# guptakhil/show-tell

Hardware: AMD Instinct MI355X
Metric: training images/sec (ResNet101+GRU, emb=512, bs=128) at 1/2/4/8 MI355X (higher is better)
Workload: dtype bf16; 1 GPU; BASELINE configs[1]: ResNet-101 (train-mode BN, frozen) + 5-layer GRU decoder, E=H=512, V=10000, fwd+bwd+SGD step, synthetic COCO-shaped batch; batch_per_gpu=128, global_batch=128, image=3x224x224, parallelism=dp1

## Files before the change

include/showtell_hip.h:

```cpp
#ifndef SHOWTELL_HIP_H
#define SHOWTELL_HIP_H

#include <stddef.h>
#include <stdint.h>

#ifdef __cplusplus
extern "C" {
#endif

#define ST_F32 0
#define ST_BF16 1

#define ST_CELL_GRU 0
#define ST_CELL_LSTM 1

const char* st_last_error(void);
int st_version(void);

typedef struct {
  const void* x;
  const void* w;
  void* y;
  const float* bias;
  const float* scale;
  const float* shift;
  const void* residual;
  float* stats;
  int dtype, out_dtype;
  int B, Hin, Win, Cin, Ho, Wo, N, KH, KW, stride, pad;
  int ldx, ldw, ldy;
  int relu, accumulate;
  int Cin_logical;
  int k_order;
  int stats_replicas;
  const float* in_stats; const float* in_gamma; const float* in_beta; float in_count, in_eps;
  int split_k;
} st_conv_desc;

int st_conv(const st_conv_desc* d, void* stream);
int st_conv_batch(const st_conv_desc* d, int n, void* stream);

typedef struct {
  const void* a;
  const void* b;
  float* c;
  const int* b_row;
  const int* b_live;
  float* colsum0;
  float* colsum1;
  int dtype;
  int M, N, K;
  int lda, ldb, ldc;
  int accumulate;
} st_gemm_tn_desc;
int st_gemm_tn_batch(const st_gemm_tn_desc* d, int n, void* stream);

typedef struct {
  const void* x; const void* w_frag; void* y;
  float* stats; int stats_replicas;
  const float* scale; const float* shift; int relu;
  const float* in_stats; const float* in_gamma; const float* in_beta; float in_count; float in_eps;
  int B, H, W, C, N;
  int in_stats_replicas;
} st_conv3x3_img_desc;
int st_conv3x3_img_supported(int H, int W, int C, int N);
int st_conv3x3_img(const st_conv3x3_img_desc* d, void* stream);
int st_conv3x3_s2_supported(int C, int N);
int st_conv3x3_s2(const st_conv3x3_img_desc* d, void* stream);
typedef struct {
  const void* x; const void* w_frag; void* y; const void* residual;
  float* stats; int stats_replicas;
  const float* scale; const float* shift; int relu;
  const float* in_stats; const float* in_gamma; const float* in_beta; float in_count; float in_eps; int in_stats_replicas;
  int B, Hin, Win, C, N, stride;
} st_conv1x1_wreg_desc;
int st_conv1x1_wreg_supported(int C, int N);
int st_conv1x1_wreg(const st_conv1x1_wreg_desc* d, void* stream);
int st_conv1x1_kstream_supported(int C, int N);
int st_conv1x1_kstream(const st_conv1x1_wreg_desc* d, void* stream);
typedef struct {
  const void* raw; const void* identity; void* x_out; const void* w_frag; void* y;
  float* stats; int stats_replicas;
  const float* f_stats; const float* f_gamma; const float* f_beta; float f_count; float f_eps; int f_stats_replicas;
  long rows; int C, N;
  const float* id_stats; const float* id_gamma; const float* id_beta; int id_stats_replicas;
} st_conv1x1_kfuse_desc;
int st_conv1x1_kfuse_supported(int C, int N);
int st_conv1x1_kfuse(const st_conv1x1_kfuse_desc* d, void* stream);
#ifdef ST_EXPERIMENTAL
int st_conv1x1_kfuse8(const st_conv1x1_kfuse_desc* d, void* stream);
#endif
typedef struct {
  const void* raw2; const void* w3_frag; const void* identity; void* x_out; const void* w1_frag; void* y;
  float* stats; int stats_replicas;
  const float* bn2_stats; const float* bn2_gamma; const float* bn2_beta; int bn2_replicas;
  const float* bn3_stats; const float* bn3_gamma; const float* bn3_beta; int bn3_replicas;
  const float* id_stats; const float* id_gamma; const float* id_beta; int id_replicas;
  float count; float eps;
  long rows; int C1, C2, N;
} st_conv_b2b_desc;
int st_conv_b2b_supported(int C1, int C2, int N);
int st_conv_b2b(const st_conv_b2b_desc* d, void* stream);
typedef struct {
  const void* x2; const void* w3_frag; const void* identity; void* x_out; const void* w1_frag; void* y;
  float* stats; int stats_replicas;
  const float* bn2_stats; const float* bn2_gamma; const float* bn2_beta; int bn2_replicas;
  const float* bn3_stats; const float* bn3_gamma; const float* bn3_beta; int bn3_replicas;
  float count; float eps;
  const float* scale3; const float* shift3; const float* scale1; const float* shift1; int relu1;
  long rows; int C1, C2, N;
  const float* id_stats; const float* id_gamma; const float* id_beta; int id_replicas;
} st_conv_c3c1_desc;
int st_conv_c3c1_supported(int C1, int C2, int N);
int st_conv_c3c1(const st_conv_c3c1_desc* d, void* stream);
int st_conv1x1_astat_supported(int C, int N);
int st_conv1x1_astat(const st_conv1x1_wreg_desc* d, void* stream);

int st_pack_conv_weight_frag(const float* w, void* out, int Cout, int Cin, int KH, int KW, int ntw, void* stream);

int st_tune(int reserved, int kc, int w8);
int st_prof_enable(int on);
int st_debug_stamps(unsigned long long* buf);
int st_prof_collect(double* ms, double* flops, long* launches);

typedef struct {
  const void* x; void* y; const void* res;
  const float* stats;  const float* gamma; const float* beta;
  const float* running_mean; const float* running_var;
  const float* res_stats; const float* res_gamma; const float* res_beta;
  const float* res_running_mean; const float* res_running_var;
  int res_bn;
  int dtype; long rows; int C; float count; float eps; int relu;
  int stats_replicas, res_stats_replicas;
} st_bn_act_desc;

int st_bn_act(const st_bn_act_desc* d, void* stream);

int st_bn_update_running(const float* stats, float* running_mean, float* running_var,
// ... 255 lines not shown
```

show-tell_amd/_lib.py:

```python
import ctypes as C
import os

import torch

_HERE = os.path.dirname(os.path.abspath(__file__))
LIB_PATH = os.path.join(_HERE, "lib", "libshowtell_hip.so")

ST_F32, ST_BF16 = 0, 1
ST_CELL_GRU, ST_CELL_LSTM = 0, 1

c_p, c_i, c_f, c_l = C.c_void_p, C.c_int, C.c_float, C.c_long


class ConvDesc(C.Structure):
    _fields_ = [("x", c_p), ("w", c_p), ("y", c_p), ("bias", c_p), ("scale", c_p), ("shift", c_p),
                ("residual", c_p), ("stats", c_p), ("dtype", c_i), ("out_dtype", c_i),
                ("B", c_i), ("Hin", c_i), ("Win", c_i), ("Cin", c_i), ("Ho", c_i), ("Wo", c_i), ("N", c_i),
                ("KH", c_i), ("KW", c_i), ("stride", c_i), ("pad", c_i),
                ("ldx", c_i), ("ldw", c_i), ("ldy", c_i), ("relu", c_i), ("accumulate", c_i), ("Cin_logical", c_i), ("k_order", c_i), ("stats_replicas", c_i),
                ("in_stats", c_p), ("in_gamma", c_p), ("in_beta", c_p), ("in_count", c_f), ("in_eps", c_f), ("split_k", c_i)]


class Conv3x3ImgDesc(C.Structure):
    _fields_ = [("x", c_p), ("w_frag", c_p), ("y", c_p), ("stats", c_p), ("stats_replicas", c_i), ("scale", c_p), ("shift", c_p),
# ... 19 lines not shown
                ("scale", c_p), ("shift", c_p), ("B", c_i), ("H", c_i), ("W", c_i)]


class ConvB2bDesc(C.Structure):
    _fields_ = [("raw2", c_p), ("w3_frag", c_p), ("identity", c_p), ("x_out", c_p), ("w1_frag", c_p), ("y", c_p),
                ("stats", c_p), ("stats_replicas", c_i),
                ("bn2_stats", c_p), ("bn2_gamma", c_p), ("bn2_beta", c_p), ("bn2_replicas", c_i),
                ("bn3_stats", c_p), ("bn3_gamma", c_p), ("bn3_beta", c_p), ("bn3_replicas", c_i),
                ("id_stats", c_p), ("id_gamma", c_p), ("id_beta", c_p), ("id_replicas", c_i),
                ("count", c_f), ("eps", c_f), ("rows", c_l), ("C1", c_i), ("C2", c_i), ("N", c_i)]


class ConvC3c1Desc(C.Structure):
    _fields_ = [("x2", c_p), ("w3_frag", c_p), ("identity", c_p), ("x_out", c_p), ("w1_frag", c_p), ("y", c_p),
                ("stats", c_p), ("stats_replicas", c_i),
                ("bn2_stats", c_p), ("bn2_gamma", c_p), ("bn2_beta", c_p), ("bn2_replicas", c_i),
                ("bn3_stats", c_p), ("bn3_gamma", c_p), ("bn3_beta", c_p), ("bn3_replicas", c_i),
                ("count", c_f), ("eps", c_f),
                ("scale3", c_p), ("shift3", c_p), ("scale1", c_p), ("shift1", c_p), ("relu1", c_i),
                ("rows", c_l), ("C1", c_i), ("C2", c_i), ("N", c_i),
                ("id_stats", c_p), ("id_gamma", c_p), ("id_beta", c_p), ("id_replicas", c_i)]


class BnActDesc(C.Structure):
    _fields_ = [("x", c_p), ("y", c_p), ("res", c_p), ("stats", c_p), ("gamma", c_p), ("beta", c_p),
                ("running_mean", c_p), ("running_var", c_p), ("res_stats", c_p), ("res_gamma", c_p),
                ("res_beta", c_p), ("res_running_mean", c_p), ("res_running_var", c_p), ("res_bn", c_i),
                ("dtype", c_i), ("rows", c_l), ("C", c_i), ("count", c_f), ("eps", c_f), ("relu", c_i),
                ("stats_replicas", c_i), ("res_stats_replicas", c_i)]


ST_MAX_LAYERS = 8


class RnnParams(C.Structure):
    _fields_ = [("cell", c_i), ("dtype", c_i), ("L", c_i), ("in0", c_i), ("H", c_i), ("V", c_i), ("E", c_i),
                ("emb", c_p), ("w_ih", c_p * ST_MAX_LAYERS), ("w_hh", c_p * ST_MAX_LAYERS),
                ("b_ih", c_p * ST_MAX_LAYERS), ("b_hh", c_p * ST_MAX_LAYERS), ("w_lin", c_p), ("b_lin", c_p)]


class RnnGrads(C.Structure):
    _fields_ = [("emb", c_p), ("w_ih", c_p * ST_MAX_LAYERS), ("w_hh", c_p * ST_MAX_LAYERS),
                ("b_ih", c_p * ST_MAX_LAYERS), ("b_hh", c_p * ST_MAX_LAYERS), ("w_lin", c_p), ("b_lin", c_p)]


class AttnParams(C.Structure):
    _fields_ = [("rnn", RnnParams), ("F", c_i), ("A", c_i), ("P", c_i),
                ("w_enc", c_p), ("b_enc", c_p), ("w_dec", c_p), ("b_dec", c_p), ("w_full", c_p), ("b_full", c_p),
                ("w_init_h", c_p), ("b_init_h", c_p), ("w_init_c", c_p), ("b_init_c", c_p), ("w_embed", c_p), ("b_embed", c_p)]


class AttnGrads(C.Structure):
    _fields_ = [("rnn", RnnGrads)] + [(n, c_p) for n in ("w_enc", "b_enc", "w_dec", "b_dec", "w_full", "b_full", "w_init_h", "b_init_h",
                                                        "w_init_c", "b_init_c", "w_embed", "b_embed")]


class PackedSeq(C.Structure):
    _fields_ = [("B", c_i), ("T", c_i), ("ntok", c_i), ("Tcap", c_i), ("batch_sizes_host", C.POINTER(c_i)),
                ("rows_b", c_p), ("rows_t", c_p), ("prev_row", c_p), ("caption", c_p)]


class DropoutDesc(C.Structure):
    _fields_ = [("p_in", C.c_double), ("p_layer", C.c_double), ("p_out", C.c_double), ("seed", c_l), ("step", c_i),
                ("buf", c_p), ("buf_bytes", C.c_size_t)]


class LossTerms(C.Structure):
    _fields_ = [("row_weight", c_p), ("nll_out", c_p), ("smoothing", c_i), ("label_smoothing", c_f), ("smooth_out", c_p),
                ("tile_sums", c_p), ("tile_sums_bytes", C.c_size_t)]


class ImageBatchDesc(C.Structure):
    _fields_ = [("src", c_p), ("src_bytes", C.c_int64), ("offset", c_p), ("height", c_p), ("width", c_p), ("flip", c_p), ("batch", c_i),
                ("max_height", c_i), ("max_width", c_i), ("out_h", c_i), ("out_w", c_i), ("lut", c_p), ("tmp", c_p),
                ("out", c_p), ("out_u8", c_p)]


_SIGS = {
    "st_version": ([], c_i),
    "st_image_transform": ([C.POINTER(ImageBatchDesc), c_p], c_i),
    "st_conv": ([C.POINTER(ConvDesc), c_p], c_i),
    "st_conv_batch": ([C.POINTER(ConvDesc), c_i, c_p], c_i),
    "st_gemm_tn_batch": ([c_p, c_i, c_p], c_i),
    "st_conv3x3_img_supported": ([c_i, c_i, c_i, c_i], c_i),
    "st_conv3x3_img": ([C.POINTER(Conv3x3ImgDesc), c_p], c_i),
    "st_conv3x3_s2_supported": ([c_i, c_i], c_i),
    "st_conv3x3_s2": ([C.POINTER(Conv3x3ImgDesc), c_p], c_i),
    "st_conv1x1_wreg_supported": ([c_i, c_i], c_i),
    "st_conv1x1_wreg": ([C.POINTER(Conv1x1WregDesc), c_p], c_i),
    "st_conv1x1_kfuse": ([C.POINTER(Conv1x1KfuseDesc), c_p], c_i),
    "st_conv1x1_kfuse_supported": ([c_i, c_i], c_i),
    "st_conv1x1_kfuse8": ([C.POINTER(Conv1x1KfuseDesc), c_p], c_i),
    "st_conv_b2b": ([C.POINTER(ConvB2bDesc), c_p], c_i),
    "st_conv_b2b_supported": ([c_i, c_i, c_i], c_i),
    "st_conv_c3c1": ([C.POINTER(ConvC3c1Desc), c_p], c_i),
    "st_conv_c3c1_supported": ([c_i, c_i, c_i], c_i),
    "st_conv1x1_astat_supported": ([c_i, c_i], c_i),
    "st_conv1x1_astat": ([C.POINTER(Conv1x1WregDesc), c_p], c_i),
    "st_conv1x1_kstream_supported": ([c_i, c_i], c_i),
    "st_conv1x1_kstream": ([C.POINTER(Conv1x1WregDesc), c_p], c_i),
    "st_pack_conv_weight_frag": ([c_p, c_p, c_i, c_i, c_i, c_i, c_i, c_p], c_i),
    "st_tune": ([c_i, c_i, c_i], c_i),
    "st_prof_enable": ([c_i], c_i),
    "st_debug_stamps": ([c_p], c_i),
    "st_prof_collect": ([C.POINTER(C.c_double), C.POINTER(C.c_double), C.POINTER(c_l)], c_i),
    "st_bn_act": ([C.POINTER(BnActDesc), c_p], c_i),
    "st_bn_update_running": ([c_p, c_p, c_p, c_i, c_f, c_f, c_p], c_i),
    "st_nchw_to_nhwc": ([c_p, c_p, c_i, c_i, c_i, c_i, c_i, c_i, c_p], c_i),
    "st_nchw_to_s2d16": ([c_p, c_p, c_i, c_i, c_i, c_i, c_p], c_i),
    "st_stem_weight_s2d": ([c_p, c_p, c_i, c_i, c_p], c_i),
    "st_stem_weight_frag": ([c_p, c_p, c_p], c_i),
    "st_stem_weight_frag_packed": ([c_p, c_i, c_p, c_p], c_i),
    "st_stem_conv_pool": ([C.POINTER(StemConvPoolDesc), c_p], c_i),
    "st_nhwc_to_ncp_f32": ([c_p, c_p, c_i, c_i, c_i, c_i, c_p], c_i),
    "st_maxpool3x3s2": ([c_p, c_p, c_i, c_i, c_i, c_i, c_i, c_p], c_i),
    "st_maxpool3x3s2_bn": ([c_p, c_p, c_i, c_i, c_i, c_i, c_i, c_p, c_p, c_p, c_p, c_p, c_f, c_f, c_p], c_i),
    "st_global_avgpool": ([c_p, c_p, c_i, c_i, c_i, c_i, c_i, c_p], c_i),
    "st_cast": ([c_p, c_p, c_i, c_i, c_l, c_p], c_i),
    "st_transpose": ([c_p, c_p, c_i, c_i, c_i, c_i, c_i, c_p], c_i),
    "st_transpose_colsum": ([c_p, c_p, c_p, c_i, c_i, c_i, c_i, c_i, c_p], c_i),
    "st_transpose_batch": ([c_p, c_p, c_p, c_i, c_i, c_i, c_i, c_i, c_i, c_p, c_p, c_p], c_i),
    "st_pack_conv_weight": ([c_p, c_p, c_i, c_i, c_i, c_i, c_i, c_i, c_i, c_p], c_i),
    "st_cast2d": ([c_p, c_p, c_i, c_i, c_i, c_i, c_i, c_i, c_p], c_i),
    "st_rnn_vocab_ld": ([c_i], c_i),
    "st_rnn_workspace_bytes": ([C.POINTER(RnnParams), C.POINTER(PackedSeq)], C.c_size_t),
    "st_rnn_forward": ([C.POINTER(RnnParams), C.POINTER(PackedSeq), c_p, c_p, C.c_size_t, c_p, c_i, c_i, c_p, c_i, C.POINTER(DropoutDesc),
                        c_p, c_p], c_i),
    "st_rnn_backward": ([C.POINTER(RnnParams), C.POINTER(RnnGrads), C.POINTER(PackedSeq), c_p, c_i, c_p, C.c_size_t, c_p,
                         C.POINTER(DropoutDesc), c_p, c_p], c_i),
    "st_rnn_fused_loss_supported": ([C.POINTER(RnnParams)], c_i),
    "st_rnn_fused_loss_bytes": ([C.POINTER(RnnParams), C.POINTER(PackedSeq)], C.c_size_t),
    "st_rnn_fused_loss_ls_bytes": ([C.POINTER(RnnParams), C.POINTER(PackedSeq)], C.c_size_t),
    "st_rnn_fused_loss": ([C.POINTER(RnnParams), C.POINTER(PackedSeq), c_p, C.c_size_t, c_p, c_p, C.c_size_t, C.POINTER(LossTerms), c_p,
                           C.POINTER(DropoutDesc), c_p], c_i),
    "st_rnn_fused_dlogits": ([C.POINTER(RnnParams), C.POINTER(PackedSeq), c_p, C.c_size_t, c_p, c_p, c_p, C.POINTER(LossTerms), c_p, c_i,
                              C.POINTER(DropoutDesc), c_p], c_i),
    "st_dropout_rows": ([c_p, c_p, c_i, c_i, c_i, c_i, c_i, C.c_double, c_l, c_i, c_i, c_i, c_p], c_i),
    "st_rnn_dropout_bytes": ([C.POINTER(RnnParams), C.POINTER(PackedSeq)], C.c_size_t),
    "st_rnn_greedy_workspace_bytes": ([C.POINTER(RnnParams), c_i], C.c_size_t),
    "st_rnn_greedy": ([C.POINTER(RnnParams), c_p, c_i, c_i, c_p, C.c_size_t, c_p, c_p, c_p], c_i),
    "st_rnn_greedy_last_route": ([], c_i),
    "st_rnn_step": ([C.POINTER(RnnParams), c_p, c_i, c_p, c_p, c_p, c_p, c_p, c_i, c_p], c_i),
    "st_embedding_rows": ([c_p, c_p, c_p, c_i, c_i, c_i, c_i, c_i, c_p], c_i),
    "st_gather_state": ([c_p, c_p, c_p, c_i, c_i, c_i, c_i, c_i, c_p], c_i),
    "st_softmax_topk": ([c_p, c_i, c_i, c_i, c_i, c_p, c_p, c_i, c_p], c_i),
    "st_beam_select": ([c_p, c_p, c_p, c_p, c_p, c_i, c_i, c_i, c_l, c_p, c_p, c_p, c_p, c_p, c_p], c_i),
    "st_beam_ban_topk": ([c_p, c_i, c_i, c_i, c_i, c_p, c_i, c_i, c_i, c_p, c_i, c_l, c_i, c_p, c_p, c_p], c_i),
    "st_beam_select_hist": ([c_p, c_p, c_p, c_p, c_p, c_i, c_i, c_i, c_l, c_p, c_p, c_p, c_p, c_p, c_p, c_p, c_i, c_i, c_p], c_i),
    "st_sample_rows": ([c_p, c_i, c_i, c_i, c_p, c_i, c_f, c_i, c_l, c_p, c_p, c_p, c_i, c_i, c_p, c_p], c_i),
    "st_rnn_sample_workspace_bytes": ([C.POINTER(RnnParams), c_i], C.c_size_t),
    "st_rnn_sample": ([C.POINTER(RnnParams), c_p, c_i, c_i, c_p, c_f, c_i, c_l, c_p, C.c_size_t, c_p, c_p, c_p], c_i),
    "st_sample_mix_rows": ([c_p, c_i, c_i, c_i, c_p, c_i, c_f, c_i, c_p, c_i, c_f, c_p, c_i, c_l, c_p, c_i, c_p, c_p, c_p, c_p, c_i, c_i, c_p,
                            c_p], c_i),
    "st_rnn_sched_inputs_workspace_bytes": ([C.POINTER(RnnParams), c_i], C.c_size_t),
    "st_rnn_sched_inputs": ([C.POINTER(RnnParams), c_p, c_i, c_p, c_i, c_p, c_i, c_p, c_p, c_f, c_f, c_i, c_p, C.c_size_t, c_p, c_p, c_p, c_p,
                             c_p], c_i),
    "st_attn_workspace_bytes": ([c_p, c_p], C.c_size_t),
    "st_attn_forward": ([c_p, c_p, c_p, c_p, c_p, C.c_size_t, c_p, c_i, c_i, c_p, c_i, C.POINTER(DropoutDesc), c_p], c_i),
    "st_attn_backward": ([c_p, c_p, c_p, c_p, c_p, c_i, c_p, c_p, c_f, c_p, c_p, C.c_size_t, C.POINTER(DropoutDesc), c_p], c_i),
    "st_attn_dropout_bytes": ([c_p, c_p], C.c_size_t),
    "st_attn_reg_loss": ([c_p, c_i, c_i, c_i, c_f, c_p, c_p], c_i),
    "st_attn_greedy_workspace_bytes": ([c_p, c_i], C.c_size_t),
    "st_attn_greedy": ([c_p, c_p, c_i, c_i, c_l, c_p, C.c_size_t, c_p, c_p], c_i),
    "st_attn_greedy_alphas": ([c_p, c_p, c_i, c_i, c_l, c_p, C.c_size_t, c_p, c_p, c_p], c_i),
    "st_attn_sample_workspace_bytes": ([c_p, c_i], C.c_size_t),
    "st_attn_sample": ([c_p, c_p, c_i, c_i, c_l, c_p, c_f, c_i, c_l, c_p, C.c_size_t, c_p, c_p, c_p, c_p], c_i),
# ... 103 lines not shown
```

show-tell_amd/csrc/gemm_tn.hip:

```cpp
#include "common.h"
#include "tn_tile.h"
#include <string.h>
#include <type_traits>

namespace {

constexpr int kMaxGroups = 12;
constexpr int kImages = 2;
constexpr int kStep = kImages * TN_BK;
constexpr int kRowsPerThread = kStep / 16;

struct TnGroup {
  const bf16_t* a; const bf16_t* b; float* c;
  const int* b_row; const int* b_live;
  float* cs0; float* cs1;
  int M, N, K, lda, ldb, ldc, accumulate;
  int tile0, ntn;
};
struct TnArgs { TnGroup g[kMaxGroups]; int ng, ntiles; };

typedef __attribute__((ext_vector_type(4))) short s16x4;
typedef __attribute__((ext_vector_type(8))) short s16x8;
typedef __attribute__((address_space(3))) s16x4 lds_s16x4;

// ... 77 lines not shown
      const int row = r0 + 16 * i;
      const int off = (row / TN_BK) * TN_IMAGE_BYTES + tn_store_off(row % TN_BK, ch);
      *reinterpret_cast<u32x4*>(buf + off) = ra[i];
      *reinterpret_cast<u32x4*>(buf + kImages * TN_IMAGE_BYTES + off) = rb[i];
    }
    if (do_cs) {
#pragma unroll
      for (int i = 0; i < kRowsPerThread; ++i)
#pragma unroll
        for (int e = 0; e < 4; ++e) {
          cs[2 * e] += __uint_as_float(ra[i][e] << 16);
          cs[2 * e + 1] += __uint_as_float(ra[i][e] & 0xffff0000u);
        }
    }
    __syncthreads();
    if (s + 1 < nsteps) {
      load((s + 1) * kStep);
      resolve((s + 2) * kStep);
    }
#pragma unroll
    for (int im = 0; im < kImages; ++im) {
      const char* ia = buf + im * TN_IMAGE_BYTES;
      const char* ib = buf + (kImages + im) * TN_IMAGE_BYTES;
      bf16x8 fa[4], fb[4];
#pragma unroll
      for (int i = 0; i < 4; ++i) { fa[i] = tr_frag(ia, lane, 4 * wm + i); fb[i] = tr_frag(ib, lane, 4 * wn + i); }
#pragma unroll
      for (int i = 0; i < 4; ++i)
#pragma unroll
        for (int j = 0; j < 4; ++j) acc[i][j] = __builtin_amdgcn_mfma_f32_16x16x32_bf16(fa[i], fb[j], acc[i][j], 0, 0, 0);
    }
  }

  float* const cbase = g.c;
  const long ldc = g.ldc;
  const bool accumulate = g.accumulate != 0;
  auto write_c = [&](auto full_tag) {
    constexpr bool kFull = decltype(full_tag)::value;
    float* const cl = cbase + (long)(m0 + 64 * wm + 4 * (lane >> 4)) * ldc + (n0 + 64 * wn + (lane & 15));
#pragma unroll
    for (int i0 = 0; i0 < 4; i0 += 2) {
      float prior[2][4][4];
#pragma unroll
      for (int i = 0; i < 2; ++i)
#pragma unroll
        for (int r = 0; r < 4; ++r)
#pragma unroll
          for (int j = 0; j < 4; ++j) {
            const int m = m0 + 64 * wm + 16 * (i0 + i) + 4 * (lane >> 4) + r, n = n0 + 64 * wn + 16 * j + (lane & 15);
            const bool ok = kFull || (m < M && n < N);
            prior[i][r][j] = 0.f;
            if (accumulate) prior[i][r][j] = ok ? cl[(16 * (i0 + i) + r) * ldc + 16 * j] : 0.f;
          }
#pragma unroll
      for (int i = 0; i < 2; ++i)
#pragma unroll
        for (int r = 0; r < 4; ++r)
#pragma unroll
          for (int j = 0; j < 4; ++j) {
            const int m = m0 + 64 * wm + 16 * (i0 + i) + 4 * (lane >> 4) + r, n = n0 + 64 * wn + 16 * j + (lane & 15);
            if (kFull || (m < M && n < N)) cl[(16 * (i0 + i) + r) * ldc + 16 * j] = prior[i][r][j] + acc[i0 + i][j][r];
          }
    }
  };
  if (m0 + TN_COLS <= M && n0 + TN_COLS <= N) write_c(std::true_type{});
  else write_c(std::false_type{});

  if (do_cs) {
    __syncthreads();
    float* red = reinterpret_cast<float*>(&lds[0][0][0][0]);
#pragma unroll
    for (int e = 0; e < 8; ++e) red[r0 * TN_COLS + 8 * ch + e] = cs[e];
    __syncthreads();
    if (tid < TN_COLS && m0 + tid < M) {
      float sum = 0.f;
#pragma unroll
      for (int r = 0; r < 16; ++r) sum += red[r * TN_COLS + tid];
      if (g.cs0) g.cs0[m0 + tid] += sum;
      if (g.cs1) g.cs1[m0 + tid] += sum;
    }
  }
}

}

extern "C" int st_gemm_tn_batch(const st_gemm_tn_desc* d, int n, void* stream) {
  ST_CHECK(d && n >= 1 && n <= kMaxGroups, "st_gemm_tn_batch: 1..%d problems per launch", kMaxGroups);
  TnArgs args;
  memset(&args, 0, sizeof(args));
  long tiles = 0;
  for (int i = 0; i < n; ++i) {
    const st_gemm_tn_desc& p = d[i];
    ST_CHECK(p.dtype == ST_BF16, "st_gemm_tn_batch: problem %d: bf16 only (the transposed LDS read is a 16-bit one)", i);
    ST_CHECK(p.a && p.b && p.c, "st_gemm_tn_batch: problem %d: null pointer", i);
    ST_CHECK(p.M >= 1 && p.N >= 1 && p.K >= 1, "st_gemm_tn_batch: problem %d: bad shape M=%d N=%d K=%d", i, p.M, p.N, p.K);
    ST_CHECK(p.lda >= p.M && p.ldb >= p.N && p.ldc >= p.N, "st_gemm_tn_batch: problem %d: leading dimension below the extent (lda=%d M=%d ldb=%d N=%d ldc=%d)",
             i, p.lda, p.M, p.ldb, p.N, p.ldc);
    ST_CHECK(p.lda % 8 == 0 && p.ldb % 8 == 0, "st_gemm_tn_batch: problem %d: lda=%d and ldb=%d must be multiples of 8", i, p.lda, p.ldb);
    ST_CHECK(((reinterpret_cast<uintptr_t>(p.a) | reinterpret_cast<uintptr_t>(p.b)) & 15) == 0, "st_gemm_tn_batch: problem %d: a and b must be 16-byte aligned", i);
    ST_CHECK(!p.b_live || p.b_row, "st_gemm_tn_batch: problem %d: b_live goes with b_row", i);
    TnGroup& g = args.g[i];
    g.a = reinterpret_cast<const bf16_t*>(p.a); g.b = reinterpret_cast<const bf16_t*>(p.b); g.c = p.c;
    g.b_row = p.b_row; g.b_live = p.b_live; g.cs0 = p.colsum0; g.cs1 = p.colsum1;
    g.M = p.M; g.N = p.N; g.K = p.K; g.lda = p.lda; g.ldb = p.ldb; g.ldc = p.ldc; g.accumulate = p.accumulate;
    g.tile0 = (int)tiles;
    g.ntn = (p.N + TN_COLS - 1) / TN_COLS;
    tiles += (long)((p.M + TN_COLS - 1) / TN_COLS) * g.ntn;
    ST_CHECK(tiles < (1L << 24), "st_gemm_tn_batch: too many output tiles");
  }
  args.ng = n; args.ntiles = (int)tiles;
  const int grid = (int)((tiles + 7) / 8 * 8);
  hipLaunchKernelGGL(gemm_tn_kernel, dim3(grid), dim3(256), 0, reinterpret_cast<hipStream_t>(stream), args);
  ST_LAUNCH_CHECK();
  return 0;
}
```

show-tell_amd/csrc/rnn.cpp:

```cpp
#include "decoder_host.h"
#include <stdlib.h>

namespace {

struct Plan {
  int G, GH, Np, Vp, maxw;
  size_t es;
  size_t x0, y, gates, cst, dyl, dx0, dgx, dgh, dhc, dcc, tA, tB, wT, wThh, wTih, gA, gB, total;
};

Plan make_plan(const st_rnn_params* p, const st_packed_seq* s) {
  Plan q;
  q.G = p->cell == ST_CELL_GRU ? 3 : 4;
  q.GH = q.G * p->H;
  q.Np = st_up8(s->ntok);
  q.Vp = st_rnn_vocab_ld(p->V);
  q.es = st_dtype_size(p->dtype);
  q.maxw = p->in0 > p->H ? p->in0 : p->H;
  const size_t n = s->ntok, L = p->L, H = p->H;
  Arena ar;
  q.x0 = ar.take(n * p->in0 * q.es);
  q.y = ar.take(L * n * H * q.es);
  q.gates = ar.take(L * n * 4 * H * q.es);
  q.cst = ar.take(p->cell == ST_CELL_LSTM ? L * n * H * q.es : 0);
// ... 115 lines not shown
namespace {
int fused_rows(const st_rnn_params* p, const st_packed_seq* s, const void* workspace, size_t workspace_bytes, const st_loss_terms* t,
               const st_dropout* drop, const char* who, const char** ytop) {
  if (check_common(p, s, who)) return 1;
  if (st_check_loss_terms(t, who)) return 1;
  ST_CHECK(st_rnn_fused_loss_supported(p), "%s: needs bf16, H = 512 and the vocabulary projection (use st_rnn_forward's logits + st_cross_entropy)", who);
  const Plan q = make_plan(p, s);
  ST_CHECK(workspace, "%s: null pointer", who);
  ST_CHECK(workspace_bytes >= q.total, "%s: workspace / scratch too small", who);
  DropPlan dp;
  if (st_drop_plan(drop, p->L, s->ntok, p->H, p->dtype, false, who, &dp)) return 1;
  *ytop = dp.out ? dp.rows(p->L - 1) : reinterpret_cast<const char*>(workspace) + q.y + (size_t)(p->L - 1) * s->ntok * p->H * q.es;
  return 0;
}
}

extern "C" int st_rnn_fused_loss(const st_rnn_params* p, const st_packed_seq* s, const void* workspace, size_t workspace_bytes,
                                 const long* targets, float* scratch, size_t scratch_bytes, const st_loss_terms* terms, float* loss_accum,
                                 const st_dropout* drop, void* stream) {
  const st_loss_terms t = terms ? *terms : st_loss_terms{};
  const char* ytop;
  if (fused_rows(p, s, workspace, workspace_bytes, &t, drop, "st_rnn_fused_loss", &ytop)) return 1;
  ST_CHECK(targets && scratch && (loss_accum || t.nll_out || t.smooth_out) && (t.tile_sums || !t.smoothing), "st_rnn_fused_loss: null pointer");
  ST_CHECK(scratch_bytes >= st_rnn_fused_loss_bytes(p, s), "st_rnn_fused_loss: workspace / scratch too small");
  ST_CHECK(!t.smoothing || t.tile_sums_bytes >= st_rnn_fused_loss_ls_bytes(p, s), "st_rnn_fused_loss: tile_sums too small (%zu < %zu)",
           t.tile_sums_bytes, st_rnn_fused_loss_ls_bytes(p, s));
  const int n = s->ntok;
  return vocab_ce_forward(ytop, p->w_lin, p->b_lin, targets, n, p->V, scratch + 2 * (size_t)n, scratch + n, scratch, loss_accum, t.row_weight,
                          t.nll_out, reinterpret_cast<hipStream_t>(stream), t.tile_sums, t.smooth_out, t.label_smoothing);
}
extern "C" int st_rnn_fused_dlogits(const st_rnn_params* p, const st_packed_seq* s, const void* workspace, size_t workspace_bytes,
                                    const long* targets, const float* scratch, const float* grad_scale_dev, const st_loss_terms* terms,
                                    void* dlogits, int ldd, const st_dropout* drop, void* stream) {
  const st_loss_terms t = terms ? *terms : st_loss_terms{};
  const char* ytop;
  if (fused_rows(p, s, workspace, workspace_bytes, &t, drop, "st_rnn_fused_dlogits", &ytop)) return 1;
  ST_CHECK(targets && scratch && dlogits, "st_rnn_fused_dlogits: null pointer");
  return vocab_ce_dlogits(ytop, p->w_lin, p->b_lin, targets, scratch, s->ntok, p->V, dlogits, ldd, 1.0f, grad_scale_dev, t.row_weight,
                          reinterpret_cast<hipStream_t>(stream), t.smoothing != 0, t.label_smoothing);
}

extern "C" int st_rnn_backward(const st_rnn_params* p, const st_rnn_grads* g, const st_packed_seq* s, const void* dlogits, int ldd,
                               void* workspace, size_t workspace_bytes, float* dfeat, const st_dropout* drop, const long* input_ids,
                               void* stream) {
  if (check_common(p, s, "st_rnn_backward")) return 1;
  ST_CHECK(g && workspace && dlogits, "st_rnn_backward: null pointer");
  DropPlan dp;
  if (st_drop_plan(drop, p->L, s->ntok, p->H, p->dtype, false, "st_rnn_backward", &dp)) return 1;
  const Plan q = make_plan(p, s);
  ST_CHECK(workspace_bytes >= q.total, "st_rnn_backward: workspace too small (%zu < %zu)", workspace_bytes, q.total);
  hipStream_t st = reinterpret_cast<hipStream_t>(stream);
  char* ws = reinterpret_cast<char*>(workspace);
  const int dt = p->dtype, H = p->H, n = s->ntok, Np = q.Np, GH = q.GH;
  const size_t es = q.es;
  const std::vector<int> off = st_packed_offsets(s);
  const int L = p->L, T = s->T;
  auto dyl = [&](int l) { return reinterpret_cast<float*>(ws + q.dyl) + (size_t)l * n * H; };
  float* dy = dyl(L - 1);
  const char* ytop = dp.out ? dp.rows(L - 1) : ws + q.y + (size_t)(p->L - 1) * n * H * es;

  const char* env_tn = getenv("ST_WGRAD_TN");
  const bool tn = dt == ST_BF16 && !(env_tn && env_tn[0] == '0');
  st_gemm_tn_desc tg[2 * ST_MAX_LAYERS + 1];
  int ntg = 0;
  auto tn_desc = [&](const void* a, int lda, const void* b, int ldb, float* c, int rows, int cols, float* cs0, float* cs1, bool hprev) {
    st_gemm_tn_desc d;
    memset(&d, 0, sizeof(d));
    d.a = a; d.b = b; d.c = c; d.colsum0 = cs0; d.colsum1 = cs1; d.dtype = dt;
    d.M = rows; d.N = cols; d.K = n; d.lda = lda; d.ldb = ldb; d.ldc = cols; d.accumulate = 1;
    if (hprev) { d.b_row = s->prev_row; d.b_live = s->rows_t; }
    return d;
  };

  ST_CHECK(p->w_lin && g->w_lin && g->b_lin, "st_rnn_backward: vocabulary projection gradients requested without buffers");
  ST_CHECK(ldd >= st_up8(p->V) && ldd % 8 == 0 && ldd <= q.Vp, "st_rnn_backward: dlogits leading dimension %d must be a multiple of 8 in [%d, %d]",
           ldd, st_up8(p->V), q.Vp);
  if (tn) {
    tg[ntg++] = tn_desc(dlogits, ldd, ytop, H, g->w_lin, p->V, H, g->b_lin, nullptr, false);
  } else {
    if (st_transpose_colsum(dlogits, ws + q.tA, g->b_lin, dt, n, p->V, ldd, Np, stream)) return 1;
    if (st_transpose(ytop, ws + q.tB, dt, n, H, H, Np, stream)) return 1;
    if (st_gemm_nt(ws + q.tA, Np, ws + q.tB, Np, g->w_lin, H, p->V, H, Np, dt, ST_F32, nullptr, stream, 1)) return 1;
  }
  if (st_transpose(p->w_lin, ws + q.wT, dt, p->V, H, H, ldd, stream)) return 1;
  const int bk = dt == ST_BF16 ? 64 : 32;
  const int split = (ldd % (8 * bk) == 0 && ldd >= 16 * bk) ? 8 : 0;
  if (st_gemm_nt(dlogits, ldd, ws + q.wT, ldd, dy, H, n, H, ldd, dt, ST_F32, nullptr, stream, 0, split)) return 1;
  if (dp.out && dropout_rows_launch(dy, dy, ST_F32, n, H, H, H, dp.kout, L - 1, 0, st)) return 1;

  const char* x0 = ws + q.x0;
  const bool need_dx0 = dfeat || g->emb;
  float* dx0 = reinterpret_cast<float*>(ws + q.dx0);
  const bool gru = p->cell == ST_CELL_GRU;
  auto dgxl = [&](int l) { return ws + q.dgx + (size_t)l * n * GH * es; };
  auto dghl = [&](int l) { return gru ? ws + q.dgh + (size_t)l * n * GH * es : dgxl(l); };
  auto dhcl = [&](int l) { return reinterpret_cast<float*>(ws + q.dhc) + (size_t)l * s->B * H; };
  auto dccl = [&](int l) { return reinterpret_cast<float*>(ws + q.dcc) + (size_t)l * s->B * H; };
  auto wThh = [&](int l) { return ws + q.wThh + (size_t)l * H * GH * es; };
  auto wTih = [&](int l) { return ws + q.wTih + (size_t)l * q.maxw * GH * es; };
  if (hipMemsetAsync(ws + q.dhc, 0, (size_t)L * s->B * H * sizeof(float), st) != hipSuccess ||
      hipMemsetAsync(ws + q.dcc, 0, (size_t)L * s->B * H * sizeof(float), st) != hipSuccess) { st_set_error("memset failed"); return 1; }
  {
    const void* wx[2][ST_MAX_LAYERS]; void* wy[2][ST_MAX_LAYERS];
    int ni = 0;
    for (int l = 0; l < L; ++l) {
      const int in = l == 0 ? p->in0 : H;
      wx[0][l] = p->w_hh[l]; wy[0][l] = wThh(l);
      if (!(l > 0 || need_dx0)) continue;
      if (in == H) { wx[1][ni] = p->w_ih[l]; wy[1][ni] = wTih(l); ++ni; }
      else if (st_transpose(p->w_ih[l], wTih(l), dt, GH, in, in, GH, stream)) return 1;
    }
    if (st_transpose_batch(wx[0], wy[0], nullptr, L, dt, GH, H, H, GH, nullptr, nullptr, stream)) return 1;
    if (ni && st_transpose_batch(wx[1], wy[1], nullptr, ni, dt, GH, H, H, GH, nullptr, nullptr, stream)) return 1;
  }
  auto bwd_cell = [&](int l, int t, const float* dyrows) {
    const char* yl = ws + q.y + (size_t)l * n * H * es;
    const char* gl = ws + q.gates + (size_t)l * n * 4 * H * es;
    const char* cl = ws + q.cst + (size_t)l * n * H * es;
    RnnBwdCell c;
    memset(&c, 0, sizeof(c));
    c.dy = dyrows ? dyrows + (size_t)off[t] * H : nullptr; c.dhc = dhcl(l); c.dcc = dccl(l);
    c.cache = gl + (size_t)off[t] * 4 * H * es;
    c.hprev = t > 0 ? yl + (size_t)off[t - 1] * H * es : nullptr;
    c.cnew = cl + (size_t)off[t] * H * es;
    c.cprev = t > 0 ? cl + (size_t)off[t - 1] * H * es : nullptr;
    c.dgx = dgxl(l) + (size_t)off[t] * GH * es; c.dgh = dghl(l) + (size_t)off[t] * GH * es; c.Bt = s->batch_sizes_host[t];
    return c;
  };
  const char* env = getenv("ST_BPTT_FUSED");
  const bool fused = !(env && env[0] == '0') || dp.layer;
  for (int d = T + L - 2; fused && d >= 0; --d) {
    RnnBwdFused fc[ST_MAX_LAYERS];
    RnnDropArgs da;
    memset(&da, 0, sizeof(da));
    da.key = dp.klayer;
    int nf = 0;
    for (int l = d < T ? 0 : d - (T - 1); l <= d && l < L; ++l) {
      const int t = d - l;
      RnnBwdFused& f = fc[nf++];
      memset(&f, 0, sizeof(f));
      f.e = bwd_cell(l, t, l == L - 1 ? dy : nullptr);
      da.site[nf - 1] = l; da.row0[nf - 1] = off[t];
      RnnGemmArgs& a = f.g;
      a.M = f.e.Bt; a.N = H;
      if (t + 1 < T) {
        a.A = dghl(l) + (size_t)off[t + 1] * GH * es; a.W = wThh(l); a.M2 = s->batch_sizes_host[t + 1]; a.K = GH; a.lda = GH; a.ldw = GH;
      }
      if (l + 1 < L) {
        a.A2 = dgxl(l + 1) + (size_t)off[t] * GH * es; a.W2 = wTih(l + 1); a.K2 = GH; a.lda2 = GH; a.ldw2 = GH;
      }
    }
    if (dp.layer ? rnn_bwd_fused_launch_batch_drop(fc, nf, p->cell, dt, da, st) : rnn_bwd_fused_launch_batch(fc, nf, p->cell, dt, st)) return 1;
  }
  if (fused && need_dx0 && st_gemm_nt(dgxl(0), GH, wTih(0), GH, dx0, p->in0, n, p->in0, GH, dt, ST_F32, nullptr, stream)) return 1;
  for (int d = T + L - 2; !fused && d >= 0; --d) {
    RnnBwdCell gc[ST_MAX_LAYERS];
    RnnGemmArgs mc[2 * ST_MAX_LAYERS];
    int ng = 0, nm = 0;
    for (int l = d < T ? 0 : d - (T - 1); l <= d && l < L; ++l) {
      const int t = d - l;
      const int bt = s->batch_sizes_host[t];
      const int in = l == 0 ? p->in0 : H;
      gc[ng++] = bwd_cell(l, t, dyl(l));
      if (t > 0) {
        RnnGemmArgs& a = mc[nm++];
        memset(&a, 0, sizeof(a));
        a.A = dghl(l) + (size_t)off[t] * GH * es; a.W = wThh(l); a.M = bt; a.N = H; a.K = GH; a.lda = GH; a.ldw = GH;
        a.out_f32 = dhcl(l); a.ldo = H; a.accumulate = 1;
      }
      if (l > 0 || need_dx0) {
// ... 65 lines not shown
```

show-tell_amd/csrc/tn_tile.h:

```cpp
#pragma once

#if defined(__HIPCC__) || defined(__CUDACC__)
#define TN_HD __host__ __device__ __forceinline__
#else
#define TN_HD inline
#endif

constexpr int TN_BK = 32;
constexpr int TN_COLS = 128;
constexpr int TN_ROW_BYTES = 2 * TN_COLS;
constexpr int TN_IMAGE_BYTES = TN_BK * TN_ROW_BYTES;

TN_HD int tn_swz(int row) { return ((row & 3) << 2) | ((row >> 2) & 3); }

TN_HD int tn_store_off(int row, int ch) { return TN_ROW_BYTES * row + 16 * (ch ^ tn_swz(row)); }

TN_HD int tn_read_row(int lane, int h) { return 8 * (lane >> 4) + 4 * h + ((lane & 15) >> 2); }

TN_HD int tn_read_off(int lane, int c16, int h) {
  const int p = lane & 3;
  return tn_store_off(tn_read_row(lane, h), 2 * c16 + (p >> 1)) + 8 * (p & 1);
}
```

show-tell_amd/gemm_tn.py:

```python
import ctypes as C

import torch

from ._lib import ST_BF16, ShowTellHipError, check, lib, ptr, stream

c_p, c_i = C.c_void_p, C.c_int


class GemmTnDesc(C.Structure):
    _fields_ = [("a", c_p), ("b", c_p), ("c", c_p), ("b_row", c_p), ("b_live", c_p), ("colsum0", c_p), ("colsum1", c_p),
                ("dtype", c_i), ("M", c_i), ("N", c_i), ("K", c_i), ("lda", c_i), ("ldb", c_i), ("ldc", c_i), ("accumulate", c_i)]


def desc(a, b, c, M, N, K=None, b_row=None, b_live=None, colsum0=None, colsum1=None, accumulate=False):
    for t in (a, b, c):
        if not t.is_cuda or t.dim() != 2 or t.stride(1) != 1:
            raise ShowTellHipError("gemm_tn: operands must be 2-d device tensors with unit column stride")
    if a.dtype != torch.bfloat16 or b.dtype != torch.bfloat16 or c.dtype != torch.float32:
        raise ShowTellHipError("gemm_tn: a and b are bfloat16, c is float32")
    return GemmTnDesc(a=ptr(a), b=ptr(b), c=ptr(c), b_row=ptr(b_row), b_live=ptr(b_live), colsum0=ptr(colsum0), colsum1=ptr(colsum1),
                      dtype=ST_BF16, M=M, N=N, K=a.shape[0] if K is None else K, lda=a.stride(0), ldb=b.stride(0), ldc=c.stride(0),
                      accumulate=int(bool(accumulate)))


def gemm_tn_batch(descs):
    arr = (GemmTnDesc * max(len(descs), 1))(*descs)
    check(lib().st_gemm_tn_batch(arr, len(descs), stream()), "st_gemm_tn_batch")
```

Measured before the change: 32320 images/sec.

## Compute decoder dy with an NN GEMM reading w_lin directly, skipping transpose

Adds a bf16 NN GEMM kernel that multiplies dlogits by the untransposed output-projection weight. It uses transposed LDS reads for the B operand and an optional split-K path with a fold kernel that sums the partials. The decoder backward uses this kernel by default instead of transposing w_lin each step and calling the NT GEMM. This removes a full transpose of the V x H weight per iteration, at the cost of an extra partial-sum buffer write and a fold pass.

```diff
diff --git a/include/showtell_hip.h b/include/showtell_hip.h
--- a/include/showtell_hip.h
+++ b/include/showtell_hip.h
@@ -54,6 +54,10 @@
   int accumulate;
 } st_gemm_tn_desc;
 int st_gemm_tn_batch(const st_gemm_tn_desc* d, int n, void* stream);
+
+size_t st_gemm_nn_partial_bytes(int n, int N, int K);
+int st_gemm_nn(const void* a, int lda, const void* b, int ldb, float* c, int ldc, int n, int N, int K, int dtype,
+               float* partial, size_t partial_bytes, void* stream);
 
 typedef struct {
   const void* x; const void* w_frag; void* y;
diff --git a/show-tell_amd/_lib.py b/show-tell_amd/_lib.py
--- a/show-tell_amd/_lib.py
+++ b/show-tell_amd/_lib.py
@@ -125,6 +125,8 @@
     "st_conv": ([C.POINTER(ConvDesc), c_p], c_i),
     "st_conv_batch": ([C.POINTER(ConvDesc), c_i, c_p], c_i),
     "st_gemm_tn_batch": ([c_p, c_i, c_p], c_i),
+    "st_gemm_nn_partial_bytes": ([c_i, c_i, c_i], C.c_size_t),
+    "st_gemm_nn": ([c_p, c_i, c_p, c_i, c_p, c_i, c_i, c_i, c_i, c_i, c_p, C.c_size_t, c_p], c_i),
     "st_conv3x3_img_supported": ([c_i, c_i, c_i, c_i], c_i),
     "st_conv3x3_img": ([C.POINTER(Conv3x3ImgDesc), c_p], c_i),
     "st_conv3x3_s2_supported": ([c_i, c_i], c_i),
diff --git a/show-tell_amd/csrc/gemm_tn.hip b/show-tell_amd/csrc/gemm_tn.hip
--- a/show-tell_amd/csrc/gemm_tn.hip
+++ b/show-tell_amd/csrc/gemm_tn.hip
@@ -183,6 +183,172 @@
   }
 }
 
+constexpr int kNnSlices = 8;
+constexpr int kNnSplitK = 2048;
+
+struct NnArgs {
+  const bf16_t* a; const bf16_t* b; float* c; float* part;
+  int n, N, K, lda, ldb, ldc, ldp;
+  int S, steps_per_slice, ntn, ntiles;
+};
+
+__global__ __launch_bounds__(256, 2) void gemm_nn_kernel(NnArgs g) {
+  __shared__ __attribute__((aligned(16))) char lds[2][NN_IMAGE_BYTES + kImages * TN_IMAGE_BYTES];
+
+  const int per = gridDim.x >> 3;
+  const int id = (blockIdx.x & 7) * per + (blockIdx.x >> 3);
+  if (id >= g.ntiles * g.S) return;
+  const int z = id / g.ntiles, tile = id % g.ntiles;
+  const int m0 = (tile / g.ntn) * NN_ROWS, n0 = (tile % g.ntn) * TN_COLS;
+  const int n = g.n, N = g.N, K = g.K;
+  const long lda = g.lda, ldb = g.ldb;
+
+  const int tid = threadIdx.x, lane = tid & 63, wave = tid >> 6;
+  const int cha = tid & 7, ra0 = tid >> 3;
+  const int chb = tid & 15, rb0 = tid >> 4;
+  const bool b_ok = n0 + 8 * chb < N;
+  const bf16_t* ap = g.a + 8 * cha;
+  const bf16_t* bp = g.b + n0 + 8 * chb;
+
+  u32x4 ra[kRowsPerThread], rb[kRowsPerThread];
+  auto load = [&](int kbase) {
+#pragma unroll
+    for (int i = 0; i < kRowsPerThread; ++i) {
+      const int m = m0 + ra0 + 32 * i, k = kbase + rb0 + 16 * i;
+      ra[i] = u32x4{0u, 0u, 0u, 0u}; rb[i] = u32x4{0u, 0u, 0u, 0u};
+      if (m < n && kbase + 8 * cha < K) ra[i] = *reinterpret_cast<const u32x4*>(ap + m * lda + kbase);
+      if (b_ok && k < K) rb[i] = *reinterpret_cast<const u32x4*>(bp + k * ldb);
+    }
+  };
+
+  f32x4 acc[4][4];
+#pragma unroll
+  for (int i = 0; i < 4; ++i)
+#pragma unroll
+    for (int j = 0; j < 4; ++j) acc[i][j] = f32x4{0.f, 0.f, 0.f, 0.f};
+
+  const int wm = wave >> 1, wn = wave & 1;
+  const int nsteps_all = (K + kStep - 1) / kStep;
+  const int s0 = z * g.steps_per_slice;
+  const int s1 = s0 + g.steps_per_slice < nsteps_all ? s0 + g.steps_per_slice : nsteps_all;
+  load(s0 * kStep);
+  for (int s = s0; s < s1; ++s) {
+    char* buf = &lds[(s - s0) & 1][0];
+    if ((s + 1) * kStep > K) {
+      const int v = K - (s * kStep + 8 * cha);
+#pragma unroll
+      for (int i = 0; i < kRowsPerThread; ++i)
+#pragma unroll
+        for (int e = 0; e < 4; ++e)
+          ra[i][e] &= (2 * e < v ? 0x0000ffffu : 0u) | (2 * e + 1 < v ? 0xffff0000u : 0u);
+    }
+#pragma unroll
+    for (int i = 0; i < kRowsPerThread; ++i) {
+      *reinterpret_cast<u32x4*>(buf + nn_a_store_off(ra0 + 32 * i, cha)) = ra[i];
+      const int row = rb0 + 16 * i;
+      *reinterpret_cast<u32x4*>(buf + NN_IMAGE_BYTES + (row / TN_BK) * TN_IMAGE_BYTES + tn_store_off(row % TN_BK, chb)) = rb[i];
+    }
+    __syncthreads();
+    if (s + 1 < s1) load((s + 1) * kStep);
+#pragma unroll
+    for (int im = 0; im < kImages; ++im) {
+      const char* ib = buf + NN_IMAGE_BYTES + im * TN_IMAGE_BYTES;
+      bf16x8 fa[4], fb[4];
+#pragma unroll
+      for (int i = 0; i < 4; ++i) {
+        const u32x4 v = *reinterpret_cast<const u32x4*>(buf + nn_a_read_off(lane, 4 * wm + i, im));
+        fa[i] = *reinterpret_cast<const bf16x8*>(&v);
+        fb[i] = tr_frag(ib, lane, 4 * wn + i);
+      }
+#pragma unroll
+      for (int i = 0; i < 4; ++i)
+#pragma unroll
+        for (int j = 0; j < 4; ++j) acc[i][j] = __builtin_amdgcn_mfma_f32_16x16x32_bf16(fa[i], fb[j], acc[i][j], 0, 0, 0);
+    }
+  }
+
+  float* const out = g.S > 1 ? g.part + (size_t)z * n * g.ldp : g.c;
+  const long ldo = g.S > 1 ? g.ldp : g.ldc;
+  float* const ol = out + (long)(m0 + 64 * wm + 4 * (lane >> 4)) * ldo + (n0 + 64 * wn + (lane & 15));
+  const bool full = m0 + NN_ROWS <= n && n0 + TN_COLS <= N;
+#pragma unroll
+  for (int i = 0; i < 4; ++i)
+#pragma unroll
+    for (int r = 0; r < 4; ++r)
+#pragma unroll
+      for (int j = 0; j < 4; ++j) {
+        const int m = m0 + 64 * wm + 16 * i + 4 * (lane >> 4) + r, col = n0 + 64 * wn + 16 * j + (lane & 15);
+        if (full || (m < n && col < N)) ol[(16 * i + r) * ldo + 16 * j] = acc[i][j][r];
+      }
+}
+
+__global__ __launch_bounds__(256) void nn_fold_kernel(const float* __restrict__ part, float* __restrict__ c, int n, int N, int ldc, int ldp, int S, int vec) {
+  const long q = (long)blockIdx.x * 256 + threadIdx.x;
+  const int per_row = ldp >> 2;
+  if (q >= (long)n * per_row) return;
+  const int m = (int)(q / per_row), col = 4 * (int)(q % per_row);
+  const size_t slice = (size_t)n * ldp;
+  const float* p = part + (size_t)m * ldp + col;
+  f32x4 v[kNnSlices];
+#pragma unroll
+  for (int z = 0; z < kNnSlices; ++z) v[z] = *reinterpret_cast<const f32x4*>(p + (z < S ? z : 0) * slice);
+  f32x4 sum = v[0];
+#pragma unroll
+  for (int z = 1; z < kNnSlices; ++z)
+    if (z < S) sum += v[z];
+  float* o = c + (size_t)m * ldc + col;
+  if (vec) { *reinterpret_cast<f32x4*>(o) = sum; return; }
+#pragma unroll
+  for (int e = 0; e < 4; ++e)
+    if (col + e < N) o[e] = sum[e];
+}
+
+int nn_slices_wanted(int K) { return K >= kNnSplitK ? kNnSlices : 1; }
+int nn_ldp(int N) { return (N + 3) & ~3; }
+
+}
+
+extern "C" size_t st_gemm_nn_partial_bytes(int n, int N, int K) {
+  if (n < 1 || N < 1 || K < 1 || nn_slices_wanted(K) == 1) return 0;
+  return (size_t)nn_slices_wanted(K) * n * nn_ldp(N) * sizeof(float);
+}
+
+extern "C" int st_gemm_nn(const void* a, int lda, const void* b, int ldb, float* c, int ldc, int n, int N, int K, int dtype,
+                          float* partial, size_t partial_bytes, void* stream) {
+  ST_CHECK(dtype == ST_BF16, "st_gemm_nn: bf16 only (the transposed LDS read is a 16-bit one)");
+  ST_CHECK(a && b && c, "st_gemm_nn: null pointer");
+  ST_CHECK(n >= 1 && N >= 1 && K >= 1, "st_gemm_nn: bad shape n=%d N=%d K=%d", n, N, K);
+  ST_CHECK(lda >= (K + 7) / 8 * 8 && ldb >= N && ldc >= N, "st_gemm_nn: leading dimension below the extent (lda=%d K=%d ldb=%d ldc=%d N=%d)", lda, K, ldb, ldc, N);
+  ST_CHECK(lda % 8 == 0 && ldb % 8 == 0, "st_gemm_nn: lda=%d and ldb=%d must be multiples of 8", lda, ldb);
+  ST_CHECK(((reinterpret_cast<uintptr_t>(a) | reinterpret_cast<uintptr_t>(b)) & 15) == 0, "st_gemm_nn: a and b must be 16-byte aligned");
+  NnArgs g;
+  memset(&g, 0, sizeof(g));
+  g.a = reinterpret_cast<const bf16_t*>(a); g.b = reinterpret_cast<const bf16_t*>(b); g.c = c; g.part = partial;
+  g.n = n; g.N = N; g.K = K; g.lda = lda; g.ldb = ldb; g.ldc = ldc; g.ldp = nn_ldp(N);
+  g.ntn = (N + TN_COLS - 1) / TN_COLS;
+  const long tiles = (long)((n + NN_ROWS - 1) / NN_ROWS) * g.ntn;
+  ST_CHECK(tiles < (1L << 24), "st_gemm_nn: too many output tiles");
+  g.ntiles = (int)tiles;
+  const int nsteps = (K + kStep - 1) / kStep;
+  const size_t one = (size_t)n * g.ldp * sizeof(float);
+  int S = nn_slices_wanted(K);
+  if (!partial || (reinterpret_cast<uintptr_t>(partial) & 15)) S = 1;
+  else if ((size_t)S * one > partial_bytes) S = (int)(partial_bytes / one);
+  if (S > nsteps) S = nsteps;
+  if (S < 2) S = 1;
+  g.steps_per_slice = (nsteps + S - 1) / S;
+  g.S = (nsteps + g.steps_per_slice - 1) / g.steps_per_slice;
+  hipStream_t st = reinterpret_cast<hipStream_t>(stream);
+  const int grid = (int)((tiles * g.S + 7) / 8 * 8);
+  hipLaunchKernelGGL(gemm_nn_kernel, dim3(grid), dim3(256), 0, st, g);
+  ST_LAUNCH_CHECK();
+  if (g.S > 1) {
+    const long quads = (long)n * (g.ldp >> 2);
+    const int vec = N % 4 == 0 && ldc % 4 == 0 && (reinterpret_cast<uintptr_t>(c) & 15) == 0;
+    hipLaunchKernelGGL(nn_fold_kernel, dim3((unsigned)((quads + 255) / 256)), dim3(256), 0, st, partial, c, n, N, ldc, g.ldp, g.S, vec);
+    ST_LAUNCH_CHECK();
+  }
+  return 0;
 }
 
 extern "C" int st_gemm_tn_batch(const st_gemm_tn_desc* d, int n, void* stream) {
diff --git a/show-tell_amd/csrc/rnn.cpp b/show-tell_amd/csrc/rnn.cpp
--- a/show-tell_amd/csrc/rnn.cpp
+++ b/show-tell_amd/csrc/rnn.cpp
@@ -221,10 +221,17 @@
     if (st_transpose(ytop, ws + q.tB, dt, n, H, H, Np, stream)) return 1;
     if (st_gemm_nt(ws + q.tA, Np, ws + q.tB, Np, g->w_lin, H, p->V, H, Np, dt, ST_F32, nullptr, stream, 1)) return 1;
   }
-  if (st_transpose(p->w_lin, ws + q.wT, dt, p->V, H, H, ldd, stream)) return 1;
-  const int bk = dt == ST_BF16 ? 64 : 32;
-  const int split = (ldd % (8 * bk) == 0 && ldd >= 16 * bk) ? 8 : 0;
-  if (st_gemm_nt(dlogits, ldd, ws + q.wT, ldd, dy, H, n, H, ldd, dt, ST_F32, nullptr, stream, 0, split)) return 1;
+  const char* env_nn = getenv("ST_DY_NN");
+  const bool nn_aligned = ((reinterpret_cast<uintptr_t>(dlogits) | reinterpret_cast<uintptr_t>(p->w_lin)) & 15) == 0;
+  if (dt == ST_BF16 && nn_aligned && !(env_nn && env_nn[0] == '0')) {
+    const size_t ra = (size_t)(p->V > GH ? p->V : GH);
+    if (st_gemm_nn(dlogits, ldd, p->w_lin, H, dy, H, n, H, p->V, dt, reinterpret_cast<float*>(ws + q.tA), ra * Np * es, stream)) return 1;
+  } else {
+    if (st_transpose(p->w_lin, ws + q.wT, dt, p->V, H, H, ldd, stream)) return 1;
+    const int bk = dt == ST_BF16 ? 64 : 32;
+    const int split = (ldd % (8 * bk) == 0 && ldd >= 16 * bk) ? 8 : 0;
+    if (st_gemm_nt(dlogits, ldd, ws + q.wT, ldd, dy, H, n, H, ldd, dt, ST_F32, nullptr, stream, 0, split)) return 1;
+  }
   if (dp.out && dropout_rows_launch(dy, dy, ST_F32, n, H, H, H, dp.kout, L - 1, 0, st)) return 1;
 
   const char* x0 = ws + q.x0;
diff --git a/show-tell_amd/csrc/tn_tile.h b/show-tell_amd/csrc/tn_tile.h
--- a/show-tell_amd/csrc/tn_tile.h
+++ b/show-tell_amd/csrc/tn_tile.h
@@ -21,3 +21,12 @@
   const int p = lane & 3;
   return tn_store_off(tn_read_row(lane, h), 2 * c16 + (p >> 1)) + 8 * (p & 1);
 }
+
+constexpr int NN_BK = 64;
+constexpr int NN_ROWS = 128;
+constexpr int NN_ROW_BYTES = 2 * NN_BK;
+constexpr int NN_IMAGE_BYTES = NN_ROWS * NN_ROW_BYTES;
+
+TN_HD int nn_a_store_off(int row, int ch) { return NN_ROW_BYTES * row + 16 * (ch ^ ((row >> 1) & 7)); }
+
+TN_HD int nn_a_read_off(int lane, int r16, int im) { return nn_a_store_off(16 * r16 + (lane & 15), 4 * im + (lane >> 4)); }
diff --git a/show-tell_amd/gemm_tn.py b/show-tell_amd/gemm_tn.py
--- a/show-tell_amd/gemm_tn.py
+++ b/show-tell_amd/gemm_tn.py
@@ -23,6 +23,26 @@
                       accumulate=int(bool(accumulate)))
 
 
+def gemm_nn(a, b, c, K=None, N=None, partial="full"):
+    for t in (a, b, c):
+        if not t.is_cuda or t.dim() != 2 or t.stride(1) != 1:
+            raise ShowTellHipError("gemm_nn: operands must be 2-d device tensors with unit column stride")
+    if a.dtype != torch.bfloat16 or b.dtype != torch.bfloat16 or c.dtype != torch.float32:
+        raise ShowTellHipError("gemm_nn: a and b are bfloat16, c is float32")
+    n = a.shape[0]
+    K = b.shape[0] if K is None else K
+    N = b.shape[1] if N is None else N
+    if K > b.shape[0] or c.shape[0] < n:
+        raise ShowTellHipError("gemm_nn: b has fewer than K rows or c fewer rows than a")
+    if isinstance(partial, str):
+        nbytes = lib().st_gemm_nn_partial_bytes(n, N, K)
+        partial = torch.empty(nbytes // 4, dtype=torch.float32, device=a.device) if nbytes else None
+    pbytes = 0 if partial is None else partial.numel() * 4
+    check(lib().st_gemm_nn(ptr(a), a.stride(0), ptr(b), b.stride(0), ptr(c), c.stride(0), n, N, K, ST_BF16, ptr(partial), pbytes,
+                           stream()), "st_gemm_nn")
+    return c
+
+
 def gemm_tn_batch(descs):
     arr = (GemmTnDesc * max(len(descs), 1))(*descs)
     check(lib().st_gemm_tn_batch(arr, len(descs), stream()), "st_gemm_tn_batch")
```

New measurement: 32090 images/sec. No clear change (-0.7%).
